# Ipsedo/MusicGAN

Measured on AMD Instinct MI355X. Metric: spectrogram-images/sec G+D step, 2x128x128 bs64, higher is better.
Workload: dtype f32

## Files before the change

musicgan_amd/csrc/wino3x3.hip:

```cpp
#include <cstdlib>
#include <type_traits>

#include "mg_common.h"
#include "pack_kernels.h"
#include "wino_common.h"

namespace {

template <int NIW, int WC, int WT>
__global__ void __launch_bounds__(64 * WT * WC, WT == 2 ? 2 : 1) wino3x3_mfma(const WinoArgs a) {
  constexpr int TPB = WT * 16;
  constexpr int NTHR = 64 * WT * WC;
  constexpr int NITEMS = TPB * WCC;
  constexpr int NITEM = (NITEMS + NTHR - 1) / NTHR;
  constexpr int V_FLOATS = 16 * TPB * WCC;
  constexpr int U4 = WC * NIW * 512;
  constexpr int NU4 = (U4 + NTHR - 1) / NTHR;
  extern __shared__ __attribute__((aligned(16))) float smem[];
  float* Vs = smem;
  float* Us = smem + V_FLOATS;
  float* red = Us + U4 * 4;

  int tid = threadIdx.x, lane, wave, col, rq, wt, wc;
  auto thread_coords = [&]() __attribute__((always_inline)) {
    asm volatile("" : "+v"(tid));
    lane = tid & 63;
    wave = __builtin_amdgcn_readfirstlane(tid >> 6);
    col = lane & 15;
    rq = lane >> 4;
    wt = wave % WT;
    wc = wave / WT;
  };
  thread_coords();
  const int ct0 = blockIdx.y * (WC * NIW);
  const int HW = a.H * a.W;
  const int Ht = a.H >> 1, Wt = a.W >> 1;
  const int nblk = a.blocks_x * a.blocks_y * a.blocks_n;

  unsigned voffP[NITEM][4], voffE[NITEM][4];
  bool ledge[NITEM], redge[NITEM];
  int vdst[NITEM];
  int bx, by, n0;
  const float* img_base;
  unsigned img_bytes;
  auto block_geometry = [&](int item) __attribute__((always_inline)) {
    const int bid = mg_xcd_remap(item, nblk);
    bx = bid % a.blocks_x;
    const int t2 = bid / a.blocks_x;
    by = t2 % a.blocks_y;
    n0 = (t2 / a.blocks_y) * a.TBN;
    const int nimg = (a.N - n0) < a.TBN ? (a.N - n0) : a.TBN;
    img_base = a.x + (size_t)n0 * a.Cin * HW;
    img_bytes = (unsigned)nimg * (unsigned)(a.Cin * HW) * 4u;
#pragma unroll
    for (int k = 0; k < NITEM; ++k) {
      const int it = tid + k * NTHR;
      const int tl = it % TPB, cl = it / TPB;
      const int txl = tl & (a.TBW - 1);
      const int tyl = (tl >> a.lgTBW) & (a.TBH - 1);
      const int nl = tl >> (a.lgTBW + a.lgTBH);
      const int TY = by * a.TBH + tyl, TX = bx * a.TBW + txl;
      const bool ok = (it < NITEMS) && (nl < nimg) && (TY < Ht) && (TX < Wt);
      const int base = (nl * a.Cin + cl) * HW + 2 * TX;
      ledge[k] = txl == 0;
      redge[k] = txl == a.TBW - 1;
#pragma unroll
      for (int r = 0; r < 4; ++r) {
        const int Y = 2 * TY - 1 + r;
        const bool rv = ok && (Y >= 0) && (Y < a.H);
        const unsigned o = (unsigned)(base + Y * a.W) * 4u;
        voffP[k][r] = rv ? o : 0x80000000u;
        voffE[k][r] = (rv && ledge[k] && TX > 0) ? o - 4u : ((rv && redge[k] && 2 * TX + 2 < a.W) ? o + 8u : 0x80000000u);
      }
      vdst[k] = (it < NITEMS) ? (((tl >> 4) * 8 * 64 + (cl >> 1) * 16 + (tl & 15)) * 4 + (cl & 1) * 2) : -1;
    }
  };

  f32x4 acc[16][NIW];

  typedef float f32x2 __attribute__((ext_vector_type(2)));
  f32x2 rP[NITEM][4];
  float rE[NITEM][4];
  f32x4 rw[NU4];

  auto load_chunk = [&](int ch) __attribute__((always_inline)) {
    const int soff = ch * WCC * HW * 4;
    const __amdgpu_buffer_rsrc_t rsrc =
        __builtin_amdgcn_make_buffer_rsrc(const_cast<float*>(img_base), 0, (int)img_bytes, 0x00020000);
#pragma unroll
    for (int k = 0; k < NITEM; ++k) {
#pragma unroll
      for (int r = 0; r < 4; ++r) {
        rP[k][r] = __builtin_bit_cast(f32x2, __builtin_amdgcn_raw_buffer_load_b64(rsrc, (int)voffP[k][r], soff, 0));
        rE[k][r] = __builtin_bit_cast(float, __builtin_amdgcn_raw_buffer_load_b32(rsrc, (int)voffE[k][r], soff, 0));
      }
    }
    const f32x4* src = reinterpret_cast<const f32x4*>(a.up + ((size_t)ch * a.NT + ct0) * 2048);
#pragma unroll
    for (int j = 0; j < NU4; ++j)
      if (NU4 * NTHR == U4 || tid + NTHR * j < U4) rw[j] = src[tid + NTHR * j];
  };

  auto store_chunk = [&](int ch) __attribute__((always_inline)) {
    if (a.Cin - ch * WCC < WCC) {
      const int lim = a.Cin - ch * WCC;
#pragma unroll
      for (int k = 0; k < NITEM; ++k)
        if ((tid + k * NTHR) / TPB >= lim) {
#pragma unroll
          for (int r = 0; r < 4; ++r) {
            rP[k][r] = f32x2{0.f, 0.f};
            rE[k][r] = 0.f;
          }
        }
    }
#pragma unroll
    for (int k = 0; k < NITEM; ++k) {
      f32x2 E[4], P[4];
#pragma unroll
      for (int r = 0; r < 4; ++r) {
        P[r] = rP[k][r];
        const float own_x = rP[k][r][0], own_y = rP[k][r][1];
        const float fl = __builtin_bit_cast(float, __builtin_amdgcn_update_dpp(0, __builtin_bit_cast(int, own_y), 0x138, 0xf, 0xf, false));
        const float fr = __builtin_bit_cast(float, __builtin_amdgcn_update_dpp(0, __builtin_bit_cast(int, own_x), 0x130, 0xf, 0xf, false));
        E[r] = f32x2{ledge[k] ? (a.TBW > 1 ? rE[k][r] : 0.f) : fl, redge[k] ? (a.TBW > 1 ? rE[k][r] : 0.f) : fr};
      }
      f32x2 UE[4], UP[4];
      UE[0] = pk_sub(E[0], E[2]);  UP[0] = pk_sub(P[0], P[2]);
      UE[1] = E[1] + E[2];         UP[1] = P[1] + P[2];
      UE[2] = pk_sub(E[2], E[1]);  UP[2] = pk_sub(P[2], P[1]);
      UE[3] = pk_sub(E[1], E[3]);  UP[3] = pk_sub(P[1], P[3]);
      if (NITEM * NTHR == NITEMS || vdst[k] >= 0) {
        float* dst = Vs + vdst[k];
#pragma unroll
        for (int i = 0; i < 4; ++i) {
          f32x2 v03, v12;
          asm("v_pk_add_f32 %0, %1, %2 op_sel:[0,1] op_sel_hi:[1,0] neg_lo:[0,1] neg_hi:[1,0]" : "=v"(v03) : "v"(UE[i]), "v"(UP[i]));
          asm("v_pk_add_f32 %0, %1, %1 op_sel:[0,1] op_sel_hi:[1,0] neg_lo:[0,0] neg_hi:[0,1]" : "=v"(v12) : "v"(UP[i]));
          *reinterpret_cast<f32x2*>(dst + (2 * i) * 256) = v03;
          *reinterpret_cast<f32x2*>(dst + (2 * i + 1) * 256) = v12;
        }
      }
    }
    f32x4* dstw = reinterpret_cast<f32x4*>(Us);
#pragma unroll
    for (int j = 0; j < NU4; ++j)
      if (NU4 * NTHR == U4 || tid + NTHR * j < U4) dstw[tid + NTHR * j] = rw[j];
  };

  auto compute_chunk = [&]() __attribute__((always_inline)) {
    const float* va = Vs + wt * 2048 + lane * 4;
    const float* ub = Us + (wc * NIW) * 2048 + lane * 4;
    f32x4 av[2], bv[2][NIW];
    av[0] = *reinterpret_cast<const f32x4*>(va);
#pragma unroll
    for (int ni = 0; ni < NIW; ++ni) bv[0][ni] = *reinterpret_cast<const f32x4*>(ub + ni * 2048);
    __builtin_amdgcn_sched_group_barrier(0x100, 1 + NIW, 0);
#pragma unroll
    for (int cp = 0; cp < 8; ++cp) {
      const int cur = cp & 1, nxt = cur ^ 1;
      if (cp + 1 < 8) {
        av[nxt] = *reinterpret_cast<const f32x4*>(va + (cp + 1) * 256);
#pragma unroll
        for (int ni = 0; ni < NIW; ++ni) bv[nxt][ni] = *reinterpret_cast<const f32x4*>(ub + ni * 2048 + (cp + 1) * 256);
      }
#pragma unroll
      for (int ks = 0; ks < 2; ++ks)
#pragma unroll
        for (int par = 0; par < 2; ++par)
#pragma unroll
          for (int ni = 0; ni < NIW; ++ni)
            acc[2 * cp + par][ni] = __builtin_amdgcn_mfma_f32_16x16x4f32(bv[cur][ni][ks * 2 + par], av[cur][ks * 2 + par], acc[2 * cp + par][ni], 0, 0, 0);
      if (cp + 1 < 8) __builtin_amdgcn_sched_group_barrier(0x100, 1 + NIW, 0);
      __builtin_amdgcn_sched_group_barrier(0x008, 4 * NIW, 0);
    }
  };

  block_geometry(blockIdx.x);
  load_chunk(0);
#pragma nounroll
  for (int item = blockIdx.x;;) {
  const int next = item + (int)gridDim.x;
  const int ebx = bx, eby = by, en0 = n0;
#pragma unroll
  for (int c = 0; c < 16; ++c)
#pragma unroll
    for (int ni = 0; ni < NIW; ++ni) {
      typedef double f64x2 __attribute__((ext_vector_type(2)));
      acc[c][ni] = __builtin_bit_cast(f32x4, f64x2{0.0, 0.0});
    }
  for (int ch = 0; ch + 1 < a.nchunk; ++ch) {
    __syncthreads();
    store_chunk(ch);
    __syncthreads();
    load_chunk(ch + 1);
    compute_chunk();
  }
  __syncthreads();
  store_chunk(a.nchunk - 1);
  __syncthreads();
  if (WT >= 4 && next < nblk) block_geometry(next);
  load_chunk(0);
  compute_chunk();

#include "wino_epilogue.h"
  if (WT < 4 || next >= nblk) break;
  item = next;
  thread_coords();
  }
}

__global__ void wino3x3_pack_kernel(const float* __restrict__ w, float* __restrict__ up, int Co, int Ci, int dgrad, int NT,
                                    size_t total) {
  const size_t e = (size_t)blockIdx.x * blockDim.x + threadIdx.x;
  if (e < total) pack_wino3x3_elem(e, w, up, Co, Ci, dgrad, NT);
}

template <int NIW, int WC, int WT>
int launch_wino(const WinoArgs& a, dim3 grid, hipStream_t s) {
  constexpr size_t lds = wino_staged_lds(NIW, WC, WT);
  static MgPerDevice once;
  if (mg_first_use_on_device(once)) {
    (void)hipFuncSetAttribute(reinterpret_cast<const void*>(&wino3x3_mfma<NIW, WC, WT>),
                              hipFuncAttributeMaxDynamicSharedMemorySize, WINO_LDS_MAX);
  }
  hipLaunchKernelGGL((wino3x3_mfma<NIW, WC, WT>), grid, dim3(64 * WT * WC), lds, s, a);
  MG_CHECK_LAUNCH("mg_wino3x3");
  return MG_OK;
}

int wino_run(WinoArgs& a, hipStream_t s);

WinoSwitches wino_switches() {
  WinoSwitches sw;
  const char* e;
  auto set = [&e](const char* name) { return (e = getenv(name)) != nullptr; };
  if (set("MG_WINO_CFG")) sw.cfg = atoi(e);
  if (set("MG_WINO_WT")) sw.wt = atoi(e);
  if (set("MG_WINO_NARROW")) sw.narrow = false;
  if (set("MG_WINO_NARROW_WT")) sw.narrow_wt = atoi(e);
  if (set("MG_WINO_FEW")) sw.few = atoi(e) != 0;
  if (set("MG_WINO_PERSIST")) sw.persist = atoi(e) != 0;
  if (set("MG_WINO_STRIP")) sw.strip = atoi(e) == 0 ? 0 : (atoi(e) > 1 ? 2 : 1);
  if (set("MG_WINO_STRIP_NIW")) sw.strip_niw = atoi(e);
  if (set("MG_WINO_STRIP_WGS")) sw.strip_wgs = atoi(e);
  if (set("MG_WINO_STRIP_PADW")) sw.strip_padw = atof(e);
  if (set("MG_WINO_STRIP_MIN_BLOCKS")) sw.strip_min_blocks = atoll(e);
  if (set("MG_WINO_STRIP_ABLATE")) sw.strip_ablate = atoi(e) & 6;
  return sw;
}

WinoLayer wino_layer(const WinoArgs& a) { return {a.N, a.Cin, a.Cout, a.H, a.W, a.flags, a.bias != nullptr, a.y != nullptr}; }

}

extern "C" size_t mg_wino3x3_packed_floats(int Cin, int Cout) {
  return (size_t)mg_cdiv(Cin, WCC) * pack_wino_nt_padded(Cout) * 2048;
}

extern "C" int mg_wino3x3_pack(const float* w, float* up, int Co, int Ci, int dgrad, mg_stream_t stream) {
  MG_CHECK_ARG(w && up && Co > 0 && Ci > 0, "mg_wino3x3_pack: bad arguments");
  const int NT = pack_wino_nt_padded(dgrad ? Ci : Co);
  const size_t total = pack_wino3x3_threads(Co, Ci, dgrad);
  hipLaunchKernelGGL(wino3x3_pack_kernel, dim3((unsigned)((total + 255) / 256)), dim3(256), 0, (hipStream_t)stream, w, up, Co,
                     Ci, dgrad, NT, total);
  MG_CHECK_LAUNCH("mg_wino3x3_pack");
  return MG_OK;
}

extern "C" int mg_wino3x3(const float* x, const float* up, const float* bias, const float* aux, float* y, float* p, float* rn,
                          int N, int Cin, int Cout, int H, int W, int flags, float slope, mg_stream_t stream) {
  MG_CHECK_ARG(x && up && N > 0 && Cin > 0 && Cout > 0 && H > 0 && W > 0, "mg_wino3x3: bad arguments");
  MG_CHECK_ARG((H % 2 == 0) && (W % 2 == 0), "mg_wino3x3: H=%d W=%d must be even", H, W);
  MG_CHECK_ARG(Cout <= 160, "mg_wino3x3: Cout=%d > 160 unsupported", Cout);
  const bool pn = flags & MG_CONV_PIXNORM;
  MG_CHECK_ARG(!(flags & MG_CONV_UPS_IN), "mg_wino3x3: UPS_IN unsupported (use mg_upconv3x3)");
  MG_CHECK_ARG(!(flags & MG_CONV_MASK_AUX) || aux, "mg_wino3x3: MASK_AUX without aux");
  MG_CHECK_ARG(!pn || ((flags & MG_CONV_LRELU) && p), "mg_wino3x3: PIXNORM needs LRELU and p");
  const bool mask_bytes = flags & MG_CONV_MASK_BYTES, mask_out = flags & MG_CONV_MASK_OUT, unpool = flags & MG_CONV_UNPOOL;
  MG_CHECK_ARG(pn || y || mask_bytes, "mg_wino3x3: y is NULL");
  MG_CHECK_ARG(!mask_out || ((flags & MG_CONV_POOL_OUT) && (flags & MG_CONV_LRELU) && !(flags & MG_CONV_MASK_AUX) && !unpool),
               "mg_wino3x3: MASK_OUT needs POOL_OUT and LRELU");
  MG_CHECK_ARG(!mask_bytes || ((flags & MG_CONV_MASK_AUX) && ((flags & MG_CONV_POOL_OUT) || y) && !unpool),
               "mg_wino3x3: MASK_BYTES needs MASK_AUX and an output (POOL_OUT: the pooled result only; else y)");
  MG_CHECK_ARG(!unpool || (aux && y && !(flags & ~MG_CONV_UNPOOL) && !bias), "mg_wino3x3: UNPOOL takes aux and y and no other flag");
  MG_CHECK_ARG(!(flags & MG_CONV_POOL_OUT) || (!pn && p), "mg_wino3x3: POOL_OUT needs p and no PIXNORM");
  MG_CHECK_ARG(!((flags & MG_CONV_MASK_AUX) && (flags & (MG_CONV_LRELU | MG_CONV_PIXNORM))),
               "mg_wino3x3: MASK_AUX excludes LRELU/PIXNORM");
  MG_CHECK_ARG(!(flags & ~(MG_CONV_LRELU | MG_CONV_PIXNORM | MG_CONV_MASK_AUX | MG_CONV_POOL_OUT | MG_CONV_MASK_OUT |
                           MG_CONV_MASK_BYTES | MG_CONV_UNPOOL)), "mg_wino3x3: unknown flag");
  MG_CHECK_ARG((long long)N * Cin * H * W < (1ll << 40) && (long long)N * Cout * H * W < (1ll << 40), "mg_wino3x3: tensor too large");
  MG_CHECK_ARG(!pn || mg_cdiv(Cout, 16) <= 4, "mg_wino3x3: PIXNORM needs Cout <= 64 (all channels of a pixel in one workgroup)");

  WinoArgs a;
  a.x = x; a.up = up; a.bias = bias; a.aux = aux; a.y = y; a.p = p; a.rn = rn;
  a.mi = reinterpret_cast<const unsigned char*>(aux);
  a.mo = reinterpret_cast<unsigned char*>(y);
  a.other = nullptr; a.coef = nullptr;
  a.N = N; a.Cin = Cin; a.Cout = Cout; a.H = H; a.W = W;
  a.flags = flags; a.slope = slope;
  return wino_run(a, (hipStream_t)stream);
}

extern "C" int mg_wino3x3_mask_bytes_y_supported(int N, int Cin, int Cout, int H, int W) {
  return wino_mask_bytes_y_supported(N, Cin, Cout, H, W, wino_switches()) ? 1 : 0;
}

namespace {
int wino_run(WinoArgs& a, hipStream_t s) {
  const WinoSwitches sw = wino_switches();
  const WinoLayer L = wino_layer(a);
  WinoStripPlan sp = wino_strip_form(L, sw);
  if (sp.takes) return mgi_wino_strip_run(a, sp, L, sw, s);
  const WinoStagedPlan p = wino_staged_plan(L, mg_cu_count(), sw);
  MG_CHECK_ARG(p.status != WINO_MASK_BYTES_SHAPE,
               "mg_wino3x3: MASK_BYTES without POOL_OUT needs a shape the strip kernel takes (N=%d %d->%d @%dx%d)", a.N, a.Cin, a.Cout,
               a.H, a.W);
  MG_CHECK_ARG(p.status != WINO_TILE_ERROR, "mg_wino3x3: internal tile error");
  MG_CHECK_ARG(p.status != WINO_BLOCK_TOO_LARGE, "mg_wino3x3: image block too large for 32-bit offsets");
  a.nchunk = p.nchunk; a.NT = p.NT;
  a.TBW = p.TBW; a.TBH = p.TBH; a.TBN = p.TBN; a.lgTBW = p.lgTBW; a.lgTBH = p.lgTBH;
  a.blocks_x = p.blocks_x; a.blocks_y = p.blocks_y; a.blocks_n = p.blocks_n;
  const dim3 grid(p.grid_x, p.grid_y);
  switch (p.cfg * 10 + p.wt) {
    case 18: return launch_wino<1, 1, 8>(a, grid, s);
    case 14: return launch_wino<1, 1, 4>(a, grid, s);
    case 12: return launch_wino<1, 1, 2>(a, grid, s);
    case 44: return launch_wino<2, 2, 4>(a, grid, s);
    case 42: return launch_wino<2, 2, 2>(a, grid, s);
    case 34: return launch_wino<1, 3, 4>(a, grid, s);
    case 32: return launch_wino<1, 3, 2>(a, grid, s);
    case 24: return launch_wino<1, 2, 4>(a, grid, s);
    case 22: return launch_wino<1, 2, 2>(a, grid, s);
  }
  mg_set_error("mg_wino3x3: no kernel for %d out-channel tiles x %d tile groups per workgroup", p.cfg, p.wt);
  return MG_EINVAL;
}
}

extern "C" int mg_wino3x3_fade(const float* x, const float* up, const float* bias, const unsigned char* mask_in, const float* other,
                               const float* coef, float* y, void* out2, int N, int Cin, int Cout, int H, int W, int mode,
                               float slope, mg_stream_t stream) {
  MG_CHECK_ARG(x && up && other && coef && y && N > 0 && Cin > 0 && Cout > 0 && H > 0 && W > 0, "mg_wino3x3_fade: bad arguments");
  MG_CHECK_ARG((H % 2 == 0) && (W % 2 == 0), "mg_wino3x3_fade: H=%d W=%d must be even", H, W);
  MG_CHECK_ARG(Cout <= 160, "mg_wino3x3_fade: Cout=%d > 160 unsupported", Cout);
  MG_CHECK_ARG(mode == MG_FADE_FWD || mode == MG_FADE_TANGENT || mode == MG_FADE_BWD, "mg_wino3x3_fade: unknown mode %d", mode);
  MG_CHECK_ARG(mode == MG_FADE_FWD ? (out2 != nullptr && mask_in == nullptr) : mask_in != nullptr,
               "mg_wino3x3_fade: FWD writes a tile mask to out2, TANGENT / BWD read mask_in");
  MG_CHECK_ARG(mode != MG_FADE_BWD || (out2 != nullptr && bias == nullptr), "mg_wino3x3_fade: BWD needs out2 and no bias");
  MG_CHECK_ARG((long long)N * Cin * H * W < (1ll << 40) && (long long)N * Cout * H * W < (1ll << 40), "mg_wino3x3_fade: tensor too large");
  WinoArgs a;
  a.x = x; a.up = up; a.bias = bias; a.aux = nullptr; a.y = y; a.rn = nullptr;
  a.p = mode == MG_FADE_BWD ? static_cast<float*>(out2) : nullptr;
  a.mi = mask_in;
  a.mo = mode == MG_FADE_FWD ? static_cast<unsigned char*>(out2) : nullptr;
  a.other = other; a.coef = coef;
  a.N = N; a.Cin = Cin; a.Cout = Cout; a.H = H; a.W = W;
  a.flags = mode == MG_FADE_FWD ? (WF_BLEND | MG_CONV_LRELU)
          : mode == MG_FADE_TANGENT ? (WF_BLEND | MG_CONV_MASK_AUX | MG_CONV_MASK_BYTES) : WF_BLEND_BWD;
  a.slope = slope;
  return wino_run(a, (hipStream_t)stream);
}
```

musicgan_amd/csrc/wino_epilogue.h:

```cpp
  const float slope_eff = (a.flags & MG_CONV_LRELU) ? a.slope : 1.0f;
  const int tl = wt * 16 + col;
  const int txl = tl & (a.TBW - 1);
  const int tyl = (tl >> a.lgTBW) & (a.TBH - 1);
  const int nl = tl >> (a.lgTBW + a.lgTBH);
  const int n = en0 + nl, TY = eby * a.TBH + tyl, TX = ebx * a.TBW + txl;
  const bool tok = (n < a.N) && (TY < Ht) && (TX < Wt);
  const int oc0 = (ct0 + wc * NIW) * 16 + rq * 4;
  const size_t pix0 = ((size_t)n * a.Cout * a.H + 2 * TY) * a.W + 2 * TX;
  const size_t pp0 = ((size_t)n * a.Cout * Ht + TY) * Wt + TX;

  auto transform = [&](int ni, float (&on)[4][4], auto act_) __attribute__((always_inline)) {
    constexpr bool ACT = decltype(act_)::value;
    f32x4 bv4;
#pragma unroll
    for (int g = 0; g < 4; ++g) {
      const int oc = oc0 + ni * 16 + g;
      bv4[g] = (a.bias != nullptr && oc < a.Cout) ? a.bias[oc] : 0.f;
    }
    constexpr int SL[4] = {0, 2, 3, 1};
    f32x4 s0[4], s1[4];
#pragma unroll
    for (int nu = 0; nu < 4; ++nu) {
      const f32x4 m0 = acc[SL[nu]][ni], m1 = acc[4 + SL[nu]][ni], m2 = acc[8 + SL[nu]][ni], m3 = acc[12 + SL[nu]][ni];
      s0[nu] = (m0 + m1) + m2;
      s1[nu] = (m1 - m2) - m3;
    }
    f32x4 r4[4];
    r4[0] = (s0[0] + s0[1]) + s0[2];
    r4[1] = (s0[1] - s0[2]) - s0[3];
    r4[2] = (s1[0] + s1[1]) + s1[2];
    r4[3] = (s1[1] - s1[2]) - s1[3];
#pragma unroll
    for (int q = 0; q < 4; ++q) {
      if constexpr (ACT) {
        const f32x4 v = r4[q] + bv4;
        const f32x4 w = v * slope_eff;
#pragma unroll
        for (int g = 0; g < 4; ++g) on[g][q] = fmaxf(v[g], w[g]);
      } else {
#pragma unroll
        for (int g = 0; g < 4; ++g) on[g][q] = r4[q][g];
      }
    }
  };
  const bool odd = (lane & 1) != 0;
  const bool wide = (a.TBW >= 2) && ((Wt & 1) == 0);
  auto swap1 = [&](float x) __attribute__((always_inline)) {
    return __builtin_bit_cast(float, __builtin_amdgcn_update_dpp(0, __builtin_bit_cast(int, x), 0xB1, 0xf, 0xf, false));
  };
  const size_t pixw = odd ? pix0 - 2 + a.W : pix0;
  auto store_tile = [&](int ni, float (&on)[4][4], const float (&rnv)[4], auto mask_, auto pn_, auto pool_, auto hasy_,
                        auto mout_, auto blend_) __attribute__((always_inline)) {
    constexpr int MASKK = decltype(mask_)::value;
    constexpr bool MASK = MASKK == 1, PN = decltype(pn_)::value, POOL = decltype(pool_)::value,
                   HASY = decltype(hasy_)::value, MOUT = decltype(mout_)::value, BLEND = decltype(blend_)::value;
    float bca = 1.f, bcb = 0.f;
    if constexpr (BLEND) { bca = a.coef[0]; bcb = a.coef[1]; }
    if constexpr (MASKK == 2 || MOUT) {
#pragma unroll
      for (int g = 0; g < 4; ++g) {
        const int oc = oc0 + ni * 16 + g;
        const bool act = tok && oc < a.Cout;
        const size_t ti = pp0 + (size_t)oc * (Ht * Wt);
        if constexpr (MASKK == 2) {
          const unsigned mb = act ? (unsigned)a.mi[ti] : 15u;
#pragma unroll
          for (int q = 0; q < 4; ++q) on[g][q] *= ((mb >> q) & 1u) ? 1.f : a.slope;
        }
        if constexpr (MOUT) {
          const unsigned mb = ((mg_pos_bit(on[g][0]) | (mg_pos_bit(on[g][1]) << 1)) | (mg_pos_bit(on[g][2]) << 2)) | (mg_pos_bit(on[g][3]) << 3);
          if (act) a.mo[ti] = (unsigned char)mb;
        }
      }
    }
    if (wide) {
      f32x4 rnw = f32x4{1.f, 1.f, 1.f, 1.f};
      if constexpr (PN) {
        const float r0 = swap1(odd ? rnv[0] : rnv[2]), r1 = swap1(odd ? rnv[1] : rnv[3]);
        rnw = odd ? f32x4{r0, r1, rnv[2], rnv[3]} : f32x4{rnv[0], rnv[1], r0, r1};
      }
#pragma unroll
      for (int g = 0; g < 4; ++g) {
        const int oc = oc0 + ni * 16 + g;
        const bool act = tok && oc < a.Cout;
        const float r0 = swap1(odd ? on[g][0] : on[g][2]), r1 = swap1(odd ? on[g][1] : on[g][3]);
        f32x4 v = odd ? f32x4{r0, r1, on[g][2], on[g][3]} : f32x4{on[g][0], on[g][1], r0, r1};
        const size_t idx = pixw + (size_t)oc * HW;
        if constexpr (MASK) {
          f32x4 ax = f32x4{1.f, 1.f, 1.f, 1.f};
          if (act) ax = *reinterpret_cast<const f32x4*>(a.aux + idx);
#pragma unroll
          for (int e = 0; e < 4; ++e) v[e] *= mg_lrelu_mask(ax[e], a.slope);
        }
        if constexpr (BLEND) {
          f32x4 o4 = f32x4{0.f, 0.f, 0.f, 0.f};
          if (act) o4 = *reinterpret_cast<const f32x4*>(a.other + idx);
          v = bca * v + bcb * o4;
        }
        float pooled = 0.f;
        if constexpr (POOL) {
          const float pe = v[0] + v[1], po = v[2] + v[3];
          pooled = ((odd ? po : pe) + swap1(odd ? pe : po)) * 0.25f;
        }
        if (act) {
          if constexpr (HASY) *reinterpret_cast<f32x4*>(a.y + idx) = v;
          if constexpr (PN) *reinterpret_cast<f32x4*>(a.p + idx) = v * rnw;
          if constexpr (POOL) a.p[pp0 + (size_t)oc * (Ht * Wt)] = pooled;
        }
      }
      return;
    }
#pragma unroll
    for (int g = 0; g < 4; ++g) {
      const int oc = oc0 + ni * 16 + g;
      if (tok && oc < a.Cout) {
        const size_t idx0 = pix0 + (size_t)oc * HW;
        float2 v0 = make_float2(on[g][0], on[g][1]), v1 = make_float2(on[g][2], on[g][3]);
        if constexpr (MASK) {
          const float2 a0 = *reinterpret_cast<const float2*>(a.aux + idx0);
          const float2 a1 = *reinterpret_cast<const float2*>(a.aux + idx0 + a.W);
          v0.x *= mg_lrelu_mask(a0.x, a.slope);
          v0.y *= mg_lrelu_mask(a0.y, a.slope);
          v1.x *= mg_lrelu_mask(a1.x, a.slope);
          v1.y *= mg_lrelu_mask(a1.y, a.slope);
        }
        if constexpr (BLEND) {
          const float2 o0 = *reinterpret_cast<const float2*>(a.other + idx0);
          const float2 o1 = *reinterpret_cast<const float2*>(a.other + idx0 + a.W);
          v0 = make_float2(bca * v0.x + bcb * o0.x, bca * v0.y + bcb * o0.y);
          v1 = make_float2(bca * v1.x + bcb * o1.x, bca * v1.y + bcb * o1.y);
        }
        if constexpr (HASY) {
          *reinterpret_cast<float2*>(a.y + idx0) = v0;
          *reinterpret_cast<float2*>(a.y + idx0 + a.W) = v1;
        }
        if constexpr (PN) {
          *reinterpret_cast<float2*>(a.p + idx0) = make_float2(v0.x * rnv[0], v0.y * rnv[1]);
          *reinterpret_cast<float2*>(a.p + idx0 + a.W) = make_float2(v1.x * rnv[2], v1.y * rnv[3]);
        }
        if constexpr (POOL) a.p[pp0 + (size_t)oc * (Ht * Wt)] = ((v0.x + v0.y) + (v1.x + v1.y)) * 0.25f;
      }
    }
  };
  auto tail = [&](auto mask_, auto pool_, auto hasy_, auto mout_, auto blend_) __attribute__((always_inline)) {
    const float one[4] = {1.f, 1.f, 1.f, 1.f};
    constexpr bool MASKED = decltype(mask_)::value != 0;
#pragma unroll
    for (int ni = 0; ni < NIW; ++ni) {
      float on[4][4];
      if (MASKED && a.bias == nullptr) transform(ni, on, std::false_type{});
      else transform(ni, on, std::true_type{});
      store_tile(ni, on, one, mask_, std::false_type{}, pool_, hasy_, mout_, blend_);
    }
  };
  auto tail_blend_bwd = [&]() __attribute__((always_inline)) {
    const float ca = a.coef[0], cb = a.coef[1];
#pragma unroll
    for (int ni = 0; ni < NIW; ++ni) {
      float on[4][4];
      transform(ni, on, std::false_type{});
#pragma unroll
      for (int g = 0; g < 4; ++g) {
        const int oc = oc0 + ni * 16 + g;
        const bool act = tok && oc < a.Cout;
        const unsigned mb = act ? (unsigned)a.mi[pp0 + (size_t)oc * (Ht * Wt)] : 15u;
        float oa[4], ob[4];
#pragma unroll
        for (int q = 0; q < 4; ++q) {
          oa[q] = (ca * on[g][q]) * (((mb >> q) & 1u) ? 1.f : a.slope);
          ob[q] = cb * on[g][q];
        }
        if (wide) {
          const float a0 = swap1(odd ? oa[0] : oa[2]), a1 = swap1(odd ? oa[1] : oa[3]);
          const float b0 = swap1(odd ? ob[0] : ob[2]), b1 = swap1(odd ? ob[1] : ob[3]);
          const f32x4 va = odd ? f32x4{a0, a1, oa[2], oa[3]} : f32x4{oa[0], oa[1], a0, a1};
          f32x4 vb = odd ? f32x4{b0, b1, ob[2], ob[3]} : f32x4{ob[0], ob[1], b0, b1};
          if (act) {
            const size_t idx = pixw + (size_t)oc * HW;
            const f32x4 ax = *reinterpret_cast<const f32x4*>(a.other + idx);
#pragma unroll
            for (int e = 0; e < 4; ++e) vb[e] *= mg_lrelu_mask(ax[e], a.slope);
            *reinterpret_cast<f32x4*>(a.y + idx) = va;
            *reinterpret_cast<f32x4*>(a.p + idx) = vb;
          }
        } else if (act) {
          const size_t idx0 = pix0 + (size_t)oc * HW;
#pragma unroll
          for (int i = 0; i < 2; ++i) {
            const float2 ax = *reinterpret_cast<const float2*>(a.other + idx0 + (size_t)i * a.W);
            *reinterpret_cast<float2*>(a.y + idx0 + (size_t)i * a.W) = make_float2(oa[2 * i], oa[2 * i + 1]);
            *reinterpret_cast<float2*>(a.p + idx0 + (size_t)i * a.W) =
                make_float2(ob[2 * i] * mg_lrelu_mask(ax.x, a.slope), ob[2 * i + 1] * mg_lrelu_mask(ax.y, a.slope));
          }
        }
      }
    }
  };
  auto tail_unpool = [&]() __attribute__((always_inline)) {
    const unsigned char* mb = reinterpret_cast<const unsigned char*>(a.aux);
    const float qh = 0.25f, ql = 0.25f * a.slope;
    const int W2 = 2 * a.W;
#pragma unroll
    for (int ni = 0; ni < NIW; ++ni) {
      float on[4][4];
      transform(ni, on, std::false_type{});
#pragma unroll
      for (int g = 0; g < 4; ++g) {
        const int oc = oc0 + ni * 16 + g;
        const bool act = tok && oc < a.Cout;
        if (wide) {
          const float r0 = swap1(odd ? on[g][0] : on[g][2]), r1 = swap1(odd ? on[g][1] : on[g][3]);
          const f32x4 v = odd ? f32x4{r0, r1, on[g][2], on[g][3]} : f32x4{on[g][0], on[g][1], r0, r1};
          if (act) {
            const size_t idx = pixw + (size_t)oc * HW;
            const unsigned mw = *reinterpret_cast<const unsigned*>(mb + idx);
            float* dst = a.y + 4 * idx - 2 * (size_t)(2 * (TX - (odd ? 1 : 0)));
#pragma unroll
            for (int r = 0; r < 2; ++r) {
              f32x4 o[2];
#pragma unroll
              for (int e = 0; e < 4; ++e)
#pragma unroll
                for (int j = 0; j < 2; ++j) o[e >> 1][(e & 1) * 2 + j] = v[e] * (((mw >> (8 * e + 2 * r + j)) & 1u) ? qh : ql);
              *reinterpret_cast<f32x4*>(dst + (size_t)r * W2) = o[0];
              *reinterpret_cast<f32x4*>(dst + (size_t)r * W2 + 4) = o[1];
            }
          }
        } else if (act) {
          const size_t idx0 = pix0 + (size_t)oc * HW;
#pragma unroll
          for (int i = 0; i < 2; ++i) {
            const unsigned mw = *reinterpret_cast<const unsigned short*>(mb + idx0 + (size_t)i * a.W);
            float* dst = a.y + 4 * (idx0 + (size_t)i * a.W) - 2 * (size_t)(2 * TX);
#pragma unroll
            for (int r = 0; r < 2; ++r) {
              f32x4 o;
#pragma unroll
              for (int e = 0; e < 2; ++e)
#pragma unroll
                for (int j = 0; j < 2; ++j) o[e * 2 + j] = on[g][2 * i + e] * (((mw >> (8 * e + 2 * r + j)) & 1u) ? qh : ql);
              *reinterpret_cast<f32x4*>(dst + (size_t)r * W2) = o;
            }
          }
        }
      }
    }
  };
  auto tail_pn = [&](auto hasy_) __attribute__((always_inline)) {
    float o[NIW][4][4];
#pragma unroll
    for (int ni = 0; ni < NIW; ++ni) transform(ni, o[ni], std::true_type{});
    float rnv[4];
#pragma unroll
    for (int q = 0; q < 4; ++q) {
      float t = 0.f;
#pragma unroll
      for (int ni = 0; ni < NIW; ++ni)
#pragma unroll
        for (int g = 0; g < 4; ++g) t += o[ni][g][q] * o[ni][g][q];
      t += __shfl_xor(t, 16);
      t += __shfl_xor(t, 32);
      rnv[q] = t;
      if (WC > 1 && rq == 0) red[(wc * TPB + tl) * 4 + q] = t;
    }
    if (WC > 1) {
      __syncthreads();
#pragma unroll
      for (int q = 0; q < 4; ++q) {
        float t = 0.f;
#pragma unroll
        for (int w2 = 0; w2 < WC; ++w2) t += red[(w2 * TPB + tl) * 4 + q];
        rnv[q] = t;
      }
    }
#pragma unroll
    for (int q = 0; q < 4; ++q) rnv[q] = 1.0f / sqrtf(rnv[q] / (float)a.Cout + PN_EPS);
#pragma unroll
    for (int ni = 0; ni < NIW; ++ni)
      store_tile(ni, o[ni], rnv, std::integral_constant<int, 0>{}, std::true_type{}, std::false_type{}, hasy_, std::false_type{},
                 std::false_type{});
    if (tok && rq == 0 && wc == 0 && a.rn != nullptr && blockIdx.y == 0) {
      const size_t r0 = ((size_t)n * a.H + 2 * TY) * a.W + 2 * TX;
      *reinterpret_cast<float2*>(a.rn + r0) = make_float2(rnv[0], rnv[1]);
      *reinterpret_cast<float2*>(a.rn + r0 + a.W) = make_float2(rnv[2], rnv[3]);
    }
  };
  using T_ = std::true_type;
  using F_ = std::false_type;
  using I0_ = std::integral_constant<int, 0>;
  using I1_ = std::integral_constant<int, 1>;
  using I2_ = std::integral_constant<int, 2>;
  if (a.flags & MG_CONV_PIXNORM) {
    if (a.y != nullptr) tail_pn(T_{});
    else tail_pn(F_{});
  } else if (a.flags & MG_CONV_UNPOOL) {
    tail_unpool();
  } else if (a.flags & WF_BLEND_BWD) {
    tail_blend_bwd();
  } else if (a.flags & WF_BLEND) {
    if (a.flags & MG_CONV_MASK_BYTES) tail(I2_{}, F_{}, T_{}, F_{}, T_{});
    else tail(I0_{}, F_{}, T_{}, T_{}, T_{});
  } else if (a.flags & MG_CONV_MASK_AUX) {
    if (a.flags & MG_CONV_MASK_BYTES) tail(I2_{}, T_{}, F_{}, F_{}, F_{});
    else if (a.flags & MG_CONV_POOL_OUT) tail(I1_{}, T_{}, T_{}, F_{}, F_{});
    else tail(I1_{}, F_{}, T_{}, F_{}, F_{});
  } else {
    if (a.flags & MG_CONV_MASK_OUT) tail(I0_{}, T_{}, F_{}, T_{}, F_{});
    else if (a.flags & MG_CONV_POOL_OUT) tail(I0_{}, T_{}, T_{}, F_{}, F_{});
    else tail(I0_{}, F_{}, T_{}, F_{}, F_{});
  }
```

Measured before the change: 5620.

## Specialize Winograd kernel per epilogue kind and trim redundant chunk work

```diff
diff --git a/musicgan_amd/csrc/wino3x3.hip b/musicgan_amd/csrc/wino3x3.hip
--- a/musicgan_amd/csrc/wino3x3.hip
+++ b/musicgan_amd/csrc/wino3x3.hip
@@ -7,7 +7,7 @@
 
 namespace {
 
-template <int NIW, int WC, int WT>
+template <int NIW, int WC, int WT, int KIND, bool KPOOL>
 __global__ void __launch_bounds__(64 * WT * WC, WT == 2 ? 2 : 1) wino3x3_mfma(const WinoArgs a) {
   constexpr int TPB = WT * 16;
   constexpr int NTHR = 64 * WT * WC;
@@ -95,14 +95,18 @@
         rE[k][r] = __builtin_bit_cast(float, __builtin_amdgcn_raw_buffer_load_b32(rsrc, (int)voffE[k][r], soff, 0));
       }
     }
-    const f32x4* src = reinterpret_cast<const f32x4*>(a.up + ((size_t)ch * a.NT + ct0) * 2048);
+    static_assert(NU4 * NTHR == U4, "every thread copies whole pieces of the filter image");
+    const __amdgpu_buffer_rsrc_t rsrc_u = __builtin_amdgcn_make_buffer_rsrc(
+        const_cast<float*>(a.up + ((size_t)ch * a.NT + ct0) * 2048), 0, U4 * 16, 0x00020000);
+    typedef unsigned u32x4 __attribute__((ext_vector_type(4)));
 #pragma unroll
     for (int j = 0; j < NU4; ++j)
-      if (NU4 * NTHR == U4 || tid + NTHR * j < U4) rw[j] = src[tid + NTHR * j];
-  };
-
-  auto store_chunk = [&](int ch) __attribute__((always_inline)) {
-    if (a.Cin - ch * WCC < WCC) {
+      rw[j] = __builtin_bit_cast(f32x4, u32x4(__builtin_amdgcn_raw_buffer_load_b128(rsrc_u, tid * 16, NTHR * 16 * j, 0)));
+  };
+
+  auto store_chunk = [&](int ch, auto last_) __attribute__((always_inline)) {
+    constexpr bool LAST = decltype(last_)::value;
+    if (LAST && a.Cin - ch * WCC < WCC) {
       const int lim = a.Cin - ch * WCC;
 #pragma unroll
       for (int k = 0; k < NITEM; ++k)
@@ -191,16 +195,18 @@
     }
   for (int ch = 0; ch + 1 < a.nchunk; ++ch) {
     __syncthreads();
-    store_chunk(ch);
+    store_chunk(ch, std::false_type{});
     __syncthreads();
     load_chunk(ch + 1);
     compute_chunk();
   }
   __syncthreads();
-  store_chunk(a.nchunk - 1);
+  store_chunk(a.nchunk - 1, std::true_type{});
   __syncthreads();
-  if (WT >= 4 && next < nblk) block_geometry(next);
-  load_chunk(0);
+  if (WT >= 4) {
+    if (next < nblk) block_geometry(next);
+    load_chunk(0);
+  }
   compute_chunk();
 
 #include "wino_epilogue.h"
@@ -216,17 +222,43 @@
   if (e < total) pack_wino3x3_elem(e, w, up, Co, Ci, dgrad, NT);
 }
 
-template <int NIW, int WC, int WT>
-int launch_wino(const WinoArgs& a, dim3 grid, hipStream_t s) {
+template <int NIW, int WC, int WT, int KIND, bool KPOOL>
+int launch_wino_kind(const WinoArgs& a, dim3 grid, hipStream_t s) {
   constexpr size_t lds = wino_staged_lds(NIW, WC, WT);
   static MgPerDevice once;
   if (mg_first_use_on_device(once)) {
-    (void)hipFuncSetAttribute(reinterpret_cast<const void*>(&wino3x3_mfma<NIW, WC, WT>),
+    (void)hipFuncSetAttribute(reinterpret_cast<const void*>(&wino3x3_mfma<NIW, WC, WT, KIND, KPOOL>),
                               hipFuncAttributeMaxDynamicSharedMemorySize, WINO_LDS_MAX);
   }
-  hipLaunchKernelGGL((wino3x3_mfma<NIW, WC, WT>), grid, dim3(64 * WT * WC), lds, s, a);
+  hipLaunchKernelGGL((wino3x3_mfma<NIW, WC, WT, KIND, KPOOL>), grid, dim3(64 * WT * WC), lds, s, a);
   MG_CHECK_LAUNCH("mg_wino3x3");
   return MG_OK;
+}
+
+template <int NIW, int WC, int WT>
+int launch_wino(const WinoArgs& a, dim3 grid, hipStream_t s) {
+  if constexpr (NIW * WC == 1 && WT > 2) {
+    return launch_wino_kind<NIW, WC, WT, -1, false>(a, grid, s);
+  } else {
+    const int kind = wino_strip_kind(a.flags);
+    const bool pool = wino_strip_pool(kind, a.flags);
+    switch (kind) {
+      case SK_ACT: return pool ? launch_wino_kind<NIW, WC, WT, SK_ACT, true>(a, grid, s) : launch_wino_kind<NIW, WC, WT, SK_ACT, false>(a, grid, s);
+      case SK_ACT_POOL_MOUT: return launch_wino_kind<NIW, WC, WT, SK_ACT_POOL_MOUT, true>(a, grid, s);
+      case SK_MB_POOL: return launch_wino_kind<NIW, WC, WT, SK_MB_POOL, true>(a, grid, s);
+      case SK_MASKF: return pool ? launch_wino_kind<NIW, WC, WT, SK_MASKF, true>(a, grid, s) : launch_wino_kind<NIW, WC, WT, SK_MASKF, false>(a, grid, s);
+      case SK_UNPOOL: return launch_wino_kind<NIW, WC, WT, SK_UNPOOL, false>(a, grid, s);
+      case SK_BLEND_FWD: return launch_wino_kind<NIW, WC, WT, SK_BLEND_FWD, false>(a, grid, s);
+      case SK_BLEND_TAN: return launch_wino_kind<NIW, WC, WT, SK_BLEND_TAN, false>(a, grid, s);
+      case SK_BLEND_BWD: return launch_wino_kind<NIW, WC, WT, SK_BLEND_BWD, false>(a, grid, s);
+      case SK_PN:
+        if constexpr (NIW * WC >= 2)
+          return a.y != nullptr ? launch_wino_kind<NIW, WC, WT, SK_PN, true>(a, grid, s) : launch_wino_kind<NIW, WC, WT, SK_PN, false>(a, grid, s);
+        break;
+    }
+    mg_set_error("mg_wino3x3: no staged kernel for epilogue kind %d with %d out-channel tiles per workgroup", kind, NIW * WC);
+    return MG_EINVAL;
+  }
 }
 
 int wino_run(WinoArgs& a, hipStream_t s);
diff --git a/musicgan_amd/csrc/wino_epilogue.h b/musicgan_amd/csrc/wino_epilogue.h
--- a/musicgan_amd/csrc/wino_epilogue.h
+++ b/musicgan_amd/csrc/wino_epilogue.h
@@ -9,6 +9,12 @@
   const size_t pix0 = ((size_t)n * a.Cout * a.H + 2 * TY) * a.W + 2 * TX;
   const size_t pp0 = ((size_t)n * a.Cout * Ht + TY) * Wt + TX;
 
+  auto mfma_results = [&](int ni) __attribute__((always_inline)) {
+    asm volatile("s_nop 7\n\ts_nop 7" : "+v"(acc[0][ni]), "+v"(acc[1][ni]), "+v"(acc[2][ni]), "+v"(acc[3][ni]), "+v"(acc[4][ni]),
+                 "+v"(acc[5][ni]), "+v"(acc[6][ni]), "+v"(acc[7][ni]));
+    asm volatile("" : "+v"(acc[8][ni]), "+v"(acc[9][ni]), "+v"(acc[10][ni]), "+v"(acc[11][ni]), "+v"(acc[12][ni]), "+v"(acc[13][ni]),
+                 "+v"(acc[14][ni]), "+v"(acc[15][ni]));
+  };
   auto transform = [&](int ni, float (&on)[4][4], auto act_) __attribute__((always_inline)) {
     constexpr bool ACT = decltype(act_)::value;
     f32x4 bv4;
@@ -23,13 +29,14 @@
     for (int nu = 0; nu < 4; ++nu) {
       const f32x4 m0 = acc[SL[nu]][ni], m1 = acc[4 + SL[nu]][ni], m2 = acc[8 + SL[nu]][ni], m3 = acc[12 + SL[nu]][ni];
       s0[nu] = (m0 + m1) + m2;
-      s1[nu] = (m1 - m2) - m3;
+      s1[nu] = pk_sub4(pk_sub4(m1, m2), m3);
     }
     f32x4 r4[4];
     r4[0] = (s0[0] + s0[1]) + s0[2];
-    r4[1] = (s0[1] - s0[2]) - s0[3];
+    r4[1] = pk_sub4(pk_sub4(s0[1], s0[2]), s0[3]);
     r4[2] = (s1[0] + s1[1]) + s1[2];
-    r4[3] = (s1[1] - s1[2]) - s1[3];
+    r4[3] = pk_sub4(pk_sub4(s1[1], s1[2]), s1[3]);
+    asm volatile("s_nop 1" : "+v"(r4[1]), "+v"(r4[3]));
 #pragma unroll
     for (int q = 0; q < 4; ++q) {
       if constexpr (ACT) {
@@ -148,6 +155,7 @@
 #pragma unroll
     for (int ni = 0; ni < NIW; ++ni) {
       float on[4][4];
+      mfma_results(ni);
       if (MASKED && a.bias == nullptr) transform(ni, on, std::false_type{});
       else transform(ni, on, std::true_type{});
       store_tile(ni, on, one, mask_, std::false_type{}, pool_, hasy_, mout_, blend_);
@@ -158,6 +166,7 @@
 #pragma unroll
     for (int ni = 0; ni < NIW; ++ni) {
       float on[4][4];
+      mfma_results(ni);
       transform(ni, on, std::false_type{});
 #pragma unroll
       for (int g = 0; g < 4; ++g) {
@@ -203,6 +212,7 @@
 #pragma unroll
     for (int ni = 0; ni < NIW; ++ni) {
       float on[4][4];
+      mfma_results(ni);
       transform(ni, on, std::false_type{});
 #pragma unroll
       for (int g = 0; g < 4; ++g) {
@@ -249,7 +259,10 @@
   auto tail_pn = [&](auto hasy_) __attribute__((always_inline)) {
     float o[NIW][4][4];
 #pragma unroll
-    for (int ni = 0; ni < NIW; ++ni) transform(ni, o[ni], std::true_type{});
+    for (int ni = 0; ni < NIW; ++ni) {
+      mfma_results(ni);
+      transform(ni, o[ni], std::true_type{});
+    }
     float rnv[4];
 #pragma unroll
     for (int q = 0; q < 4; ++q) {
@@ -290,7 +303,25 @@
   using I0_ = std::integral_constant<int, 0>;
   using I1_ = std::integral_constant<int, 1>;
   using I2_ = std::integral_constant<int, 2>;
-  if (a.flags & MG_CONV_PIXNORM) {
+  if constexpr (KIND == SK_PN) {
+    tail_pn(std::integral_constant<bool, KPOOL>{});
+  } else if constexpr (KIND == SK_UNPOOL) {
+    tail_unpool();
+  } else if constexpr (KIND == SK_BLEND_BWD) {
+    tail_blend_bwd();
+  } else if constexpr (KIND == SK_BLEND_TAN) {
+    tail(I2_{}, F_{}, T_{}, F_{}, T_{});
+  } else if constexpr (KIND == SK_BLEND_FWD) {
+    tail(I0_{}, F_{}, T_{}, T_{}, T_{});
+  } else if constexpr (KIND == SK_MB_POOL) {
+    tail(I2_{}, T_{}, F_{}, F_{}, F_{});
+  } else if constexpr (KIND == SK_MASKF) {
+    tail(I1_{}, std::integral_constant<bool, KPOOL>{}, T_{}, F_{}, F_{});
+  } else if constexpr (KIND == SK_ACT_POOL_MOUT) {
+    tail(I0_{}, T_{}, F_{}, T_{}, F_{});
+  } else if constexpr (KIND == SK_ACT) {
+    tail(I0_{}, std::integral_constant<bool, KPOOL>{}, T_{}, F_{}, F_{});
+  } else if (a.flags & MG_CONV_PIXNORM) {
     if (a.y != nullptr) tail_pn(T_{});
     else tail_pn(F_{});
   } else if (a.flags & MG_CONV_UNPOOL) {
```

Measured after the change: 5640 (median of 6 runs). No clear change (+0.3%).
